# Julian-Wyatt/AnoDDPM

Measured on AMD Instinct MI355X. Metric: reverse-diffusion images/sec @256x256 T=1000 simplex, higher is better.
Workload: dtype f32; 1 GPU; 256x256 simplex(8 oct) T=1000 base128 attn16,8 batch4/GPU (BASELINE config 2); per_gpu_batch=4, global_batch=4, T=1000, parallelism=batch-sharded x1 (no data-path collective), output_finite=True

## Files before the change

anoddpm_amd/csrc/common.h:

```cpp
#pragma once
#include <hip/hip_runtime.h>
#include <stdint.h>
#include <stdio.h>
#include "../../include/anoddpm_hip.h"

namespace anoddpm {

void set_error(const char *fmt, ...);
extern int g_debug[16];

#define ANODDPM_REQUIRE(cond, ...)                       \
    do {                                                 \
        if (!(cond)) {                                   \
            ::anoddpm::set_error(__VA_ARGS__);           \
            return ANODDPM_EINVAL;                       \
        }                                                \
    } while (0)

inline int check_launch(const char *what)
{
    hipError_t e = hipGetLastError();
    if (e != hipSuccess) {
        set_error("%s: %s", what, hipGetErrorString(e));
        return ANODDPM_ELAUNCH;
    }
    return ANODDPM_OK;
}

constexpr int ANODDPM_MAX_DEV = 64;
inline int allow_big_lds(const void *fn, bool *done, const char *what)
{
    int dev = 0;
    if (hipGetDevice(&dev) != hipSuccess || dev < 0 || dev >= ANODDPM_MAX_DEV) dev = -1;
    if (dev >= 0 && done[dev]) return ANODDPM_OK;
    hipError_t e = hipFuncSetAttribute(fn, hipFuncAttributeMaxDynamicSharedMemorySize, 160 * 1024);
    if (e != hipSuccess) {
        set_error("%s: hipFuncSetAttribute(MaxDynamicSharedMemorySize): %s", what, hipGetErrorString(e));
        return ANODDPM_ELAUNCH;
    }
    if (dev >= 0) done[dev] = true;
    return ANODDPM_OK;
}

int launch_winograd(const anoddpm_igemm_args *a, hipStream_t s);
int launch_winograd43(const anoddpm_igemm_args *a, hipStream_t s);
int launch_winograd43r(const anoddpm_igemm_args *a, hipStream_t s);
int launch_winograd43w(const anoddpm_igemm_args *a, hipStream_t s, int tsplit);
int launch_pointwise_stream(const anoddpm_igemm_args *a, hipStream_t s);
int launch_smallmap(const anoddpm_igemm_args *a, hipStream_t s);
int smallmap_tile(int ks, int H, int W, int K, int c0, int N, int B);
int launch_wino23s(const anoddpm_igemm_args *a, hipStream_t s);
int launch_winograd43b(const anoddpm_igemm_args *a, hipStream_t s);
int wino23s_tile(int H, int W, int K, int c0, int N, int B, int a_mode);
int launch_wgrad43(const anoddpm_wgrad_args *a, hipStream_t s);
int wgrad43_groups(int K, int N, int B, int H, int W);
int wgrad43_colsum_items(int K, int N, int B, int H, int W);

inline hipStream_t as_stream(void *s) { return reinterpret_cast<hipStream_t>(s); }

__device__ __forceinline__ float silu_f(float x)
{
    return x * __builtin_amdgcn_rcpf(1.0f + __expf(-x));
}

}
```

anoddpm_amd/csrc/winograd43.hip:

```cpp
#include "common.h"
#include "gn_fold.h"

using anoddpm::silu_f;

namespace {

typedef float f32x4 __attribute__((ext_vector_type(4)));

constexpr int F4_NT = 768;
constexpr int F4_KC = 16;
constexpr int F4_PW = 18;
constexpr int F4_PPIX = F4_PW * F4_PW;
constexpr int F4_PITCH = 5;
constexpr int F4_PJ = 2;
constexpr int F4_SLOTPX = F4_PJ * F4_NT / 4;
constexpr int F4_DT = F4_SLOTPX * F4_PITCH;
constexpr int F4_V = 36 * 16 * 4;
constexpr int F4_MS = 52;
constexpr int F4_LOOP_FLOATS = (2 * F4_DT + 2 * F4_V) * 4;
constexpr int F4_EX_FLOATS = 36 * 16 * F4_MS;
constexpr int F4_LDS_FLOATS = F4_EX_FLOATS > F4_LOOP_FLOATS ? F4_EX_FLOATS : F4_LOOP_FLOATS;
constexpr int F4_KMAX = 1024;
constexpr int F4_AFF_FLOATS = 2 * F4_KMAX;

// ... 318 lines not shown
    };
    float rv[ROUNDS][16], add[ROUNDS], cs[ROUNDS], cq[ROUNDS];
    prefetch(item_of(0), rv[0], add[0]);
#pragma unroll
    for (int round = 0; round < ROUNDS; ++round) {
        const int nt0 = round * RT;
        const int ntn = (NTL == 8 && round == 2) ? 2 : RT;
#pragma unroll
        for (int p = 0; p < 3; ++p)
#pragma unroll
            for (int nt = 0; nt < 3; ++nt)
                if (nt < ntn) {
#pragma unroll
                    for (int r = 0; r < 4; ++r)
                        M[((wave * 3 + p) * 16 + kq * 4 + r) * F4_MS + nt * 16 + l15] = acc[p][nt0 + nt][r];
                }
        __syncthreads();
        if (round + 1 < ROUNDS) prefetch(item_of(round + 1), rv[round + 1], add[round + 1]);
        const Item it = item_of(round);
        cs[round] = 0.f;
        cq[round] = 0.f;
        if (it.active) {
            const float *m = M + (size_t)it.tile * F4_MS + it.ch;
            float y[4][6];
#pragma unroll
            for (int v = 0; v < 6; ++v) {
                float mu[6];
#pragma unroll
                for (int u = 0; u < 6; ++u) mu[u] = m[(size_t)((u * 6 + v) * 16) * F4_MS];
                const float s12 = mu[1] + mu[2], d12 = mu[1] - mu[2], s34 = mu[3] + mu[4], d34 = mu[3] - mu[4];
                y[0][v] = mu[0] + s12 + s34;
                y[1][v] = d12 + 2.f * d34;
                y[2][v] = s12 + 4.f * s34;
                y[3][v] = d12 + 8.f * d34 + mu[5];
            }
#pragma unroll
            for (int i = 0; i < 4; ++i) {
                const float s12 = y[i][1] + y[i][2], d12 = y[i][1] - y[i][2], s34 = y[i][3] + y[i][4], d34 = y[i][3] - y[i][4];
                float o4[4];
                o4[0] = y[i][0] + s12 + s34;
                o4[1] = d12 + 2.f * d34;
                o4[2] = s12 + 4.f * s34;
                o4[3] = d12 + 8.f * d34 + y[i][5];
#pragma unroll
                for (int j = 0; j < 4; ++j) {
                    const unsigned so = ((unsigned)i * uW + (unsigned)j) * 4u;
                    const float v = a.alpha * o4[j] + add[round] + rv[round][i * 4 + j];
                    __builtin_amdgcn_raw_buffer_store_b32(__builtin_bit_cast(unsigned, v), rO, (int)it.vo, (int)(so * o_ld), 0);
                    cs[round] += v;
                    cq[round] += v * v;
                }
            }
        }
        __syncthreads();
    }
    if (a.stats || a.stats_csum) {
        float *rs = M, *rq = M + ROUNDS * 16 * 48;
#pragma unroll
        for (int round = 0; round < ROUNDS; ++round) {
            const Item it = item_of(round);
            if (it.active) { rs[(round * 16 + it.tile) * 48 + it.ch] = cs[round]; rq[(round * 16 + it.tile) * 48 + it.ch] = cq[round]; }
        }
        __syncthreads();
        if (tid < NTL * 16) {
            const int round = tid / (RT * 16), chl = tid - round * (RT * 16);
            float s = 0.f, q = 0.f;
#pragma unroll
            for (int t = 0; t < 16; ++t) { s += rs[(round * 16 + t) * 48 + chl]; q += rq[(round * 16 + t) * 48 + chl]; }
            if (a.stats_csum) {
                anoddpm::csum_atomic_add(a.stats_csum, b, N, n0 + tid, s, q);
            } else {
                float *st = a.stats + (((int64_t)b * gridDim.x + blockIdx.x) * N + n0 + tid) * 2;
                st[0] = s;
                st[1] = q;
            }
        }
    }
}

}

extern "C" int anoddpm_f43_channel_sliced(int32_t H, int32_t W, int32_t N, int32_t B);

namespace anoddpm {

int launch_winograd43(const anoddpm_igemm_args *a, hipStream_t s)
{
    ANODDPM_REQUIRE(a->ks == 3 && a->b_mode == 0 && a->heads == 1, "winograd43: needs a 3x3 conv with packed weights");
    ANODDPM_REQUIRE(a->ksplit == 1 || (a->N % 128 == 0 && a->ws && (int64_t)a->B * a->ksplit <= 65535), "winograd43: split-K needs N %% 128 == 0 and a workspace");
    ANODDPM_REQUIRE(a->a_mode == 0 || a->a_mode == 1, "winograd43: pooled operand loads use the direct kernel");
    ANODDPM_REQUIRE(a->H % 16 == 0 && a->W % 16 == 0 && a->N % 64 == 0, "winograd43: H, W must be multiples of 16 and N of 64");
    const int K = a->c0 + a->c1;
    ANODDPM_REQUIRE(K % F4_KC == 0 && (a->c1 == 0 || a->c0 % F4_KC == 0), "winograd43: channel counts must be multiples of 16");
    ANODDPM_REQUIRE((int64_t)36 * K * a->N * 4 < ((int64_t)1 << 31), "winograd43: transformed weights exceed 32-bit buffer offsets");
    ANODDPM_REQUIRE(!(a->gn_scale || a->fold_gamma) || K <= F4_KMAX, "winograd43: the GroupNorm affine table holds %d input channels", F4_KMAX);
    if (a->fold_gamma) {
        ANODDPM_REQUIRE(a->fold_beta && a->fold_stats0 && (a->c1 == 0 || a->fold_stats1) && a->fold_fmt0 == 1 && (a->c1 == 0 || a->fold_fmt1 == 1),
                        "winograd43: the GroupNorm fold takes fp64 sums (fold_fmt 1: stats_csum / tail_csum sources) only");
        ANODDPM_REQUIRE(a->fold_groups >= 1 && a->fold_groups <= 64 && K % a->fold_groups == 0 && a->ksplit == 1,
                        "winograd43: GroupNorm fold: bad group count, or split-K");
        ANODDPM_REQUIRE(((uintptr_t)a->fold_stats0 | (uintptr_t)a->fold_stats1 | (uintptr_t)a->fold_gamma | (uintptr_t)a->fold_beta) % 16 == 0,
                        "winograd43: GroupNorm fold: sums, gamma and beta must be 16-byte aligned");
    }
    if (a->stats_csum)
        ANODDPM_REQUIRE(!a->stats && a->ksplit == 1 && a->heads == 1, "winograd43: stats_csum excludes stats rows, split-K and heads");
    ANODDPM_REQUIRE((int64_t)a->H * a->W * (a->a0_ld > a->a1_ld ? a->a0_ld : a->a1_ld) * 4 < ((int64_t)1 << 31),
                    "winograd43: operand slice exceeds 32-bit buffer offsets");
    const int64_t wg128 = (int64_t)(a->H / 16) * (a->W / 16) * (a->N / 128) * a->B;
    const bool half = (a->N % 128 != 0) || ((2 * wg128 + 255) / 256) * 71 < ((wg128 + 255) / 256) * 100;
    ANODDPM_REQUIRE(!a->gnb_partial || (a->ksplit == 1 && anoddpm_f43_channel_sliced(a->H, a->W, a->N, a->B) == 1),
                    "winograd43: gnb_partial needs the channel-sliced 128-channel kernel (anoddpm_f43_channel_sliced) and ksplit 1");
    const int nblk = half ? 64 : 128;
    dim3 grid((unsigned)((a->H / 16) * (a->W / 16)), (unsigned)(a->N / nblk), (unsigned)a->B);
    ANODDPM_REQUIRE(a->B <= 65535, "winograd43: batch too large");
    const bool fast = (a->gn_scale || a->fold_gamma) && a->act;
    ANODDPM_REQUIRE(a->res_mode == 0 || (a->res_mode == 1 && a->res && a->ksplit == 1), "winograd43: res_mode 1 needs a residual and ksplit 1");
#ifdef ANODDPM_ABLATE
    const int dbg = anoddpm::g_debug[2];
#else
    const int dbg = 0;
#endif
    if (a->ksplit > 1) {
        const int K16 = K / F4_KC, cps = (K16 + a->ksplit - 1) / a->ksplit;
        ANODDPM_REQUIRE((a->ksplit - 1) * cps < K16, "winograd43: ksplit leaves a slice without channels");
        return launch_winograd43r(a, s);
    }
    {
        const int v5 = anoddpm::g_debug[5];
        if (dbg == 0 && a->N % 128 == 0 && ((!half && (v5 == 4 || v5 == 5 || v5 == 8 || v5 == 9)) || v5 == 6 || v5 == 7))
            return launch_winograd43w(a, s, (v5 & 1) | (v5 >= 8 ? 2 : 0));
    }
    if (dbg == 0 && ((!half && anoddpm::g_debug[5] != 1) || (a->N % 128 == 0 && anoddpm::g_debug[5] == 3))) return launch_winograd43r(a, s);
#ifdef ANODDPM_ABLATE
    if (fast && dbg == 1) hipLaunchKernelGGL((wino43_kernel<true, 1>), grid, dim3(F4_NT), 0, s, *a);
    else if (fast && dbg == 2) hipLaunchKernelGGL((wino43_kernel<true, 2>), grid, dim3(F4_NT), 0, s, *a);
    else if (fast && dbg == 3) hipLaunchKernelGGL((wino43_kernel<true, 3>), grid, dim3(F4_NT), 0, s, *a);
    else if (fast && dbg == 4) hipLaunchKernelGGL((wino43_kernel<true, 4>), grid, dim3(F4_NT), 0, s, *a);
    else
#endif
    ANODDPM_REQUIRE(half || !a->fold_gamma, "winograd43: the position-sliced 128-channel kernel (ANODDPM_DEBUG5=1) does not fold the GroupNorm");
    if (fast && half) hipLaunchKernelGGL((wino43_kernel<true, 0, 4>), grid, dim3(F4_NT), 0, s, *a);
    else if (half) hipLaunchKernelGGL((wino43_kernel<false, 0, 4>), grid, dim3(F4_NT), 0, s, *a);
    else if (fast) hipLaunchKernelGGL((wino43_kernel<true>), grid, dim3(F4_NT), 0, s, *a);
    else      hipLaunchKernelGGL((wino43_kernel<false>), grid, dim3(F4_NT), 0, s, *a);
    return check_launch("winograd43");
}

}

extern "C" int anoddpm_f43_channel_sliced(int32_t H, int32_t W, int32_t N, int32_t B)
{
    if (H <= 0 || W <= 0 || N <= 0 || B <= 0 || H % 16 || W % 16 || N % 128) return 0;
    const int64_t wg128 = (int64_t)(H / 16) * (W / 16) * (N / 128) * B;
    const bool half = ((2 * wg128 + 255) / 256) * 71 < ((wg128 + 255) / 256) * 100;
    const int v5 = anoddpm::g_debug[5];
#ifdef ANODDPM_ABLATE
    if (anoddpm::g_debug[2] != 0) return 0;
#endif
    return ((!half && v5 == 0) || v5 == 3) ? 1 : 0;
}
```

anoddpm_amd/csrc/winograd43r.hip:

```cpp
#include <type_traits>

#include "common.h"
#include "gn_fold.h"

using anoddpm::silu_f;

namespace {

typedef float f32x4 __attribute__((ext_vector_type(4)));
typedef float f32x2 __attribute__((ext_vector_type(2)));
typedef unsigned u32x4 __attribute__((ext_vector_type(4)));

constexpr int R4_NT = 512;
constexpr int R4_KC = 16;
constexpr int R4_PW = 18;
constexpr int R4_PPIX = R4_PW * R4_PW;
constexpr int R4_PITCH = 5;
constexpr int R4_PJ = 3;
constexpr int R4_SLOTPX = R4_PJ * R4_NT / 4;
constexpr int R4_DT = R4_SLOTPX * R4_PITCH;
constexpr int R4_V = 36 * 16 * 4;
constexpr int R4_KMAX = 1024;
constexpr int R4_AFF = 2 * R4_KMAX / 4;
constexpr int R4_LDS_FLOATS = (2 * R4_DT + 2 * R4_V + R4_AFF) * 4;

__device__ __forceinline__ __amdgpu_buffer_rsrc_t rsrc(const float *base)
{
    return __builtin_amdgcn_make_buffer_rsrc(const_cast<float *>(base), 0, 0x7ffffffe, 0x00020000);
}
__device__ __forceinline__ f32x4 bld4(__amdgpu_buffer_rsrc_t r, unsigned lane_bytes, unsigned wave_bytes)
{
    return __builtin_bit_cast(f32x4, __builtin_amdgcn_raw_buffer_load_b128(r, (int)lane_bytes, (int)wave_bytes, 0));
}
template <int AUX>
__device__ __forceinline__ f32x4 bld4x(__amdgpu_buffer_rsrc_t r, unsigned lane_bytes, unsigned wave_bytes)
{
    return __builtin_bit_cast(f32x4, __builtin_amdgcn_raw_buffer_load_b128(r, (int)lane_bytes, (int)wave_bytes, AUX));
}

__device__ __forceinline__ void at6(const float (&m)[6], float (&o)[4])
{
    const float s12 = m[1] + m[2], d12 = m[1] - m[2], s34 = m[3] + m[4], d34 = m[3] - m[4];
    o[0] = m[0] + s12 + s34;
    o[1] = d12 + 2.f * d34;
    o[2] = s12 + 4.f * s34;
    o[3] = d12 + 8.f * d34 + m[5];
}

#ifndef F43_PAIR_TRANSFORM
#define F43_PAIR_TRANSFORM 0
#endif
constexpr int R4_VAR = F43_PAIR_TRANSFORM ? 32 : 0;
template <bool FAST, int DBG = 0, int R4_RING = 6, int NPOS = 36, int VAR = 0, bool GNB = false>
__global__ __launch_bounds__(R4_NT, 1) void wino43r_kernel(const anoddpm_igemm_args a)
{
    constexpr bool V_DEPHASE = (VAR & 1) != 0, V_SCALAR_T = (VAR & 2) != 0;
    constexpr bool V_PAIRS = (VAR & 32) != 0;
    constexpr bool V_PAIR = (VAR & 4) != 0, V_PRIO = (VAR & 8) != 0;
    constexpr int PATCH_AUX = (DBG == 18 || DBG == 19 || DBG == 21) ? 2 : 0;
    constexpr int RES_AUX = (DBG == 19 || DBG == 21) ? 2 : 0;
    constexpr int STORE_AUX = DBG == 19 ? 2 : ((DBG == 20 || DBG == 21) ? 16 : 0);
    unsigned long long tstamp[5];
    if (DBG == 5 || DBG == 6) tstamp[0] = __builtin_amdgcn_s_memtime();
    __shared__ __attribute__((aligned(16))) float lds[R4_LDS_FLOATS];
    f32x4 *ldsD = reinterpret_cast<f32x4 *>(lds);
    f32x4 *ldsV = ldsD + 2 * R4_DT;
    f32x4 *ldsAff = ldsV + 2 * R4_V;

    const int tid = threadIdx.x, lane = tid & 63;
    const int wave = __builtin_amdgcn_readfirstlane(tid >> 6);
    const int H = a.H, W = a.W;
    const int K = a.c0 + a.c1, N = a.N, K4 = K >> 2;
    const int tiles_x = W >> 4;
    int tile = blockIdx.x;
    if ((VAR & 16) && (gridDim.x & 7) == 0) tile = (blockIdx.x & 7) * (gridDim.x >> 3) + (blockIdx.x >> 3);
    const int y0 = (tile / tiles_x) * 16, x0 = (tile % tiles_x) * 16;
    const int n0 = blockIdx.y * 128;
    const int ksplit = a.ksplit;
    const int ksi = blockIdx.z % ksplit;
    const int b = blockIdx.z / ksplit;
    const int a_mode = a.a_mode;

    const float *A0 = a.a0 + (int64_t)b * a.a0_bs;
    const float *A1 = a.a1 ? a.a1 + (int64_t)b * a.a1_bs : nullptr;
    const float *gsc = a.gn_scale ? a.gn_scale + (int64_t)b * a.gn_ld : nullptr;
    const float *gsh = a.gn_shift ? a.gn_shift + (int64_t)b * a.gn_ld : nullptr;
    const bool fold = a.fold_gamma != nullptr;
    const bool affine = gsc != nullptr || fold, act = a.act != 0;
    const int cps = (K / R4_KC + ksplit - 1) / ksplit;
    const int cb = ksi * cps;
    const int nchunks = (cb + cps <= K / R4_KC ? cps : K / R4_KC - cb);

    int spix[R4_PJ];
    const int pq = tid & 3;
#pragma unroll
    for (int j = 0; j < R4_PJ; ++j) {
        const int p = (tid + j * R4_NT) >> 2;
        const int py = p / R4_PW, px = p - py * R4_PW;
        const int gy = y0 + py - 1, gx = x0 + px - 1;
        int sp = -1;
        if (p < R4_PPIX && gy >= 0 && gy < H && gx >= 0 && gx < W)
            sp = (a_mode == 0) ? gy * W + gx : (gy >> 1) * (W >> 1) + (gx >> 1);
        spix[j] = sp;
    }
    f32x4 praw[R4_PJ];
    f32x4 asc = {1.f, 1.f, 1.f, 1.f}, ash = {0.f, 0.f, 0.f, 0.f};
    const __amdgpu_buffer_rsrc_t rA0 = rsrc(A0), rA1 = rsrc(A1 ? A1 : A0);
    const __amdgpu_buffer_rsrc_t rSc = rsrc(gsc ? gsc : A0), rSh = rsrc(gsh ? gsh : A0);
    auto load_patch = [&](int chunk) {
        const int kbase = (cb + chunk) * R4_KC;
        const bool first = kbase < a.c0;
        const __amdgpu_buffer_rsrc_t r = first ? rA0 : rA1;
        const unsigned ld = (unsigned)(first ? a.a0_ld : a.a1_ld);
        const unsigned koff = (unsigned)(first ? kbase : kbase - a.c0) * 4u;
#pragma unroll
        for (int j = 0; j < R4_PJ; ++j) {
            const unsigned sp = (DBG == 7) ? (unsigned)(y0 * W + x0) : (spix[j] >= 0 ? (unsigned)spix[j] : 0u);
            praw[j] = bld4x<PATCH_AUX>(r, (sp * ld + (unsigned)(pq * 4)) * 4u, koff);
        }
    };
    auto store_patch = [&](int buf, int chunk) {
        const f32x4 zero = {0.f, 0.f, 0.f, 0.f};
        if (FAST || affine) {
            asc = ldsAff[(cb + chunk) * 4 + pq];
            ash = ldsAff[K4 + (cb + chunk) * 4 + pq];
        }
#pragma unroll
        for (int j = 0; j < R4_PJ; ++j) {
            const int idx = tid + j * R4_NT;
            f32x4 v = praw[j];
            if (DBG == 22) {
                const f32x4 same = {0.25f, -0.5f, 0.75f, 1.0f};
                v = (praw[j][0] == 12345.678f) ? praw[j] : same;
            }
            if (FAST) {
                v = v * asc + ash;
                v[0] = silu_f(v[0]); v[1] = silu_f(v[1]); v[2] = silu_f(v[2]); v[3] = silu_f(v[3]);
            } else {
                if (affine) v = v * asc + ash;
                if (act) { v[0] = silu_f(v[0]); v[1] = silu_f(v[1]); v[2] = silu_f(v[2]); v[3] = silu_f(v[3]); }
            }
            ldsD[buf * R4_DT + (idx >> 2) * R4_PITCH + (idx & 3)] = spix[j] >= 0 ? v : zero;
        }
    };

    const int tu = wave % 6;
    const int tpair = lane & 7;
    const int ttile = ((wave / 6) * 2 + (lane >> 5)) * 4 + ((lane >> 3) & 3);
    const int tbase2 = (((4 * (ttile >> 2)) * R4_PW + 4 * (ttile & 3)) * R4_PITCH) * 2 + tpair;
    const bool two_pass = wave >= 2 && wave <= 5;
    constexpr int PASS_D = 8 * R4_PW * R4_PITCH * 2;
    constexpr int PASS_V = 8 * 8;
    const int tr0 = (tu == 0) ? 0 : 1, tr1 = (tu == 5) ? 3 : 2, tr2 = (tu == 0) ? 4 : ((tu == 5) ? 5 : 3), tr3 = 4;
    const float tc0 = (tu == 0) ? 4.f : (tu == 1 ? -4.f : (tu == 2 ? 4.f : (tu == 3 ? -2.f : (tu == 4 ? 2.f : 4.f))));
    const float tc1 = (tu == 0 || tu == 5) ? -5.f : ((tu == 1 || tu == 2) ? -4.f : -1.f);
    const float tc2 = (tu == 0 || tu == 5) ? 1.f : (tu == 1 ? 1.f : (tu == 2 ? -1.f : (tu == 3 ? 2.f : -2.f)));
    const float tc3 = (tu == 0 || tu == 5) ? 0.f : 1.f;
    const int to0 = tr0 * R4_PW * R4_PITCH * 2, to1 = tr1 * R4_PW * R4_PITCH * 2, to2 = tr2 * R4_PW * R4_PITCH * 2, to3 = tr3 * R4_PW * R4_PITCH * 2;
    auto transform = [&](int pbuf, int vbuf, int dofs, int vofs) {
        const f32x2 *D = reinterpret_cast<const f32x2 *>(ldsD + pbuf * R4_DT) + tbase2 + dofs;
// ... 9 lines not shown
        V[3 * 128] = r + 2.f * s;
        V[4 * 128] = r - 2.f * s;
        V[5 * 128] = 4.f * t[1] - 5.f * t[3] + t[5];
    };
    auto transform_s = [&](int pbuf, int vbuf, int dofs, int vofs) {
        const f32x2 *D = reinterpret_cast<const f32x2 *>(ldsD + pbuf * R4_DT) + tbase2 + dofs;
        float tx[6], ty[6];
#pragma unroll
        for (int j = 0; j < 6; ++j) {
            const f32x2 d0 = D[to0 + j * R4_PITCH * 2], d1 = D[to1 + j * R4_PITCH * 2], d2 = D[to2 + j * R4_PITCH * 2], d3 = D[to3 + j * R4_PITCH * 2];
            tx[j] = tc0 * d0[0] + tc1 * d1[0] + tc2 * d2[0] + tc3 * d3[0];
            ty[j] = tc0 * d0[1] + tc1 * d1[1] + tc2 * d2[1] + tc3 * d3[1];
        }
        f32x2 *V = reinterpret_cast<f32x2 *>(ldsV + vbuf * R4_V) + ((tu * 6) * 16 + ttile) * 8 + tpair + vofs;
        const float px = tx[4] - 4.f * tx[2], qx = tx[3] - 4.f * tx[1], rx = tx[4] - tx[2], sx = tx[3] - tx[1];
        const float py = ty[4] - 4.f * ty[2], qy = ty[3] - 4.f * ty[1], ry = ty[4] - ty[2], sy = ty[3] - ty[1];
        V[0 * 128] = f32x2{4.f * tx[0] - 5.f * tx[2] + tx[4], 4.f * ty[0] - 5.f * ty[2] + ty[4]};
        V[1 * 128] = f32x2{px + qx, py + qy};
        V[2 * 128] = f32x2{px - qx, py - qy};
        V[3 * 128] = f32x2{rx + 2.f * sx, ry + 2.f * sy};
        V[4 * 128] = f32x2{rx - 2.f * sx, ry - 2.f * sy};
        V[5 * 128] = f32x2{4.f * tx[1] - 5.f * tx[3] + tx[5], 4.f * ty[1] - 5.f * ty[3] + ty[5]};
    };
    const int p_up = wave % 3;
    const int p_tx = lane >> 4, p_ch = lane & 15;
    constexpr int PP = R4_PITCH * 4, PROW = R4_PW * PP;
    const int p_in = ((4 * (wave / 3)) * R4_PW + 4 * p_tx) * PP + p_ch;
    const int p_out = ((wave / 3) * 4 + p_tx) * 16 + p_ch;
    const int p_ua = p_up == 0 ? 0 : (p_up == 1 ? 1 : 3), p_ub = p_up == 0 ? 5 : (p_up == 1 ? 2 : 4);
    constexpr int PASS_DP = 8 * PROW, PASS_VP = 2 * 4 * 16;
    auto col_pass = [&](const float (&t)[6], float *V) {
        const float p = t[4] - 4.f * t[2], q = t[3] - 4.f * t[1], r = t[4] - t[2], w = t[3] - t[1];
        V[0 * 256] = 4.f * t[0] - 5.f * t[2] + t[4];
        V[1 * 256] = p + q;
        V[2 * 256] = p - q;
        V[3 * 256] = r + 2.f * w;
        V[4 * 256] = r - 2.f * w;
        V[5 * 256] = 4.f * t[1] - 5.f * t[3] + t[5];
    };
    auto transform_p = [&](int pbuf, int vbuf, int dofs, int vofs) {
        const float *D = reinterpret_cast<const float *>(ldsD + pbuf * R4_DT) + p_in + dofs;
        float ta[6], tb[6];
        if (p_up == 0) {
#pragma unroll
            for (int j = 0; j < 6; ++j) {
                const float d0 = D[j * PP], d1 = D[PROW + j * PP], d2 = D[2 * PROW + j * PP], d3 = D[3 * PROW + j * PP], d4 = D[4 * PROW + j * PP], d5 = D[5 * PROW + j * PP];
                ta[j] = 4.f * d0 - 5.f * d2 + d4;
                tb[j] = 4.f * d1 - 5.f * d3 + d5;
            }
        } else if (p_up == 1) {
#pragma unroll
            for (int j = 0; j < 6; ++j) {
                const float d1 = D[PROW + j * PP], d2 = D[2 * PROW + j * PP], d3 = D[3 * PROW + j * PP], d4 = D[4 * PROW + j * PP];
                const float p = d4 - 4.f * d2, q = d3 - 4.f * d1;
                ta[j] = p + q;
                tb[j] = p - q;
            }
        } else {
#pragma unroll
            for (int j = 0; j < 6; ++j) {
                const float d1 = D[PROW + j * PP], d2 = D[2 * PROW + j * PP], d3 = D[3 * PROW + j * PP], d4 = D[4 * PROW + j * PP];
                const float r = d4 - d2, w = d3 - d1;
                ta[j] = r + 2.f * w;
                tb[j] = r - 2.f * w;
            }
        }
        float *V = reinterpret_cast<float *>(ldsV + vbuf * R4_V) + p_out + vofs;
        col_pass(ta, V + p_ua * 6 * 256);
        col_pass(tb, V + p_ub * 6 * 256);
    };
    auto transform_all = [&](int pbuf, int vbuf) {
        if (V_PAIRS) {
            transform_p(pbuf, vbuf, 0, 0);
            if (two_pass) transform_p(pbuf, vbuf, PASS_DP, PASS_VP);
        } else if (V_SCALAR_T) {
            transform_s(pbuf, vbuf, 0, 0);
            if (two_pass) transform_s(pbuf, vbuf, PASS_D, PASS_V);
        } else {
            transform(pbuf, vbuf, 0, 0);
            if (two_pass) transform(pbuf, vbuf, PASS_D, PASS_V);
        }
    };

    f32x4 acc[NPOS];
#pragma unroll
    for (int p = 0; p < NPOS; ++p) acc[p] = f32x4{0.f, 0.f, 0.f, 0.f};

    const int l15 = lane & 15, kq = lane >> 4;
    const int nw = n0 + wave * 16 + l15;
    const __amdgpu_buffer_rsrc_t rU = rsrc(a.bmat);
    const unsigned xi_bytes = (unsigned)K4 * (unsigned)N * 16u;
    const unsigned ulane = ((unsigned)kq * (unsigned)N + (unsigned)nw) * 16u;
    const int vread = l15 * 4 + kq;

    f32x4 ring[R4_RING];
    auto load_b = [&](int chunk, int pos, int slot) {
        ring[slot] = bld4(rU, ulane, (unsigned)pos * xi_bytes + (unsigned)((cb + chunk) * 4) * (unsigned)N * 16u);
    };

    const int last = nchunks - 1;
    const int c1 = last >= 1 ? 1 : 0, c2 = last >= 2 ? 2 : last;
    f32x4 aff_sc = {0.f, 0.f, 0.f, 0.f}, aff_sh = {0.f, 0.f, 0.f, 0.f};
    const bool aff_slot = (FAST || affine) && tid < K4 && !fold;
    anoddpm::FoldLoads fl;
    if (aff_slot) {
        aff_sc = bld4(rSc, (unsigned)(tid * 16), 0u);
        aff_sh = bld4(rSh, (unsigned)(tid * 16), 0u);
    } else if (fold) {
        fl = anoddpm::fold_affine_request(a, b, tid);
    }
    load_patch(0);
    f32x4 praw0[R4_PJ];
#pragma unroll
    for (int j = 0; j < R4_PJ; ++j) praw0[j] = praw[j];
    load_patch(c1);
#pragma unroll
    for (int g = 0; g < R4_RING; ++g) load_b(0, g, g);
    if (FAST || affine) {
        if (fold) {
            anoddpm::fold_affine_finish(a, fl, tid, a_mode == 1 ? (H >> 1) * (W >> 1) : H * W, reinterpret_cast<double *>(ldsV), ldsAff);
        } else if (aff_slot) {
            ldsAff[tid] = aff_sc;
            ldsAff[K4 + tid] = aff_sh;
        }
        __syncthreads();
    }
    {
        f32x4 keep[R4_PJ];
#pragma unroll
        for (int j = 0; j < R4_PJ; ++j) { keep[j] = praw[j]; praw[j] = praw0[j]; }
        store_patch(0, 0);
#pragma unroll
        for (int j = 0; j < R4_PJ; ++j) praw[j] = keep[j];
    }
    __syncthreads();
    transform_all(0, 0);
    store_patch(1, c1);
    load_patch(c2);
    __syncthreads();
    if (DBG == 5 || DBG == 6) tstamp[1] = __builtin_amdgcn_s_memtime();

    auto step = [&](const int chunk, auto doT, auto doS, auto doL, auto doR, auto &&res_prefetch) {
        if (decltype(doT)::value && DBG != 2 && !(V_DEPHASE && wave >= 4)) transform_all((chunk + 1) & 1, (chunk + 1) & 1);
        const f32x4 *V = ldsV + (chunk & 1) * R4_V + vread;
        constexpr int PS = NPOS / 4, PL = 3 * NPOS / 4, PR = NPOS - 6;
        if (V_PAIR) {
            f32x4 av4[4];
            av4[0] = V[0];
            av4[1] = V[64];
#pragma unroll
            for (int p = 0; p < NPOS; p += 2) {
                if (V_DEPHASE && p == NPOS / 2 && decltype(doT)::value && wave >= 4) transform_all((chunk + 1) & 1, (chunk + 1) & 1);
                if ((p == PS || p == PS + 1) && decltype(doS)::value) store_patch(chunk & 1, chunk + 2);
                if ((p == PL || p == PL + 1) && decltype(doL)::value) load_patch(chunk + 3);
                if ((p == PR || p == PR + 1) && decltype(doR)::value) res_prefetch();
                const f32x4 a0 = av4[p % 4], a1 = av4[(p + 1) % 4];
                if (p + 2 < NPOS) { av4[(p + 2) % 4] = V[(p + 2) * 64]; av4[(p + 3) % 4] = V[(p + 3) * 64]; }
                const f32x4 b0 = ring[p % R4_RING], b1 = ring[(p + 1) % R4_RING];
#pragma unroll
                for (int kk = 0; kk < 4; ++kk) {
                    acc[p] = __builtin_amdgcn_mfma_f32_16x16x4f32(a0[kk], b0[kk], acc[p], 0, 0, 0);
                    acc[p + 1] = __builtin_amdgcn_mfma_f32_16x16x4f32(a1[kk], b1[kk], acc[p + 1], 0, 0, 0);
                }
#pragma unroll
                for (int q = p; q < p + 2; ++q) {
                    if (q + R4_RING < NPOS)           load_b(chunk, q + R4_RING, q % R4_RING);
                    else if (!decltype(doR)::value)   load_b(chunk + 1, q + R4_RING - NPOS, q % R4_RING);
                }
                __builtin_amdgcn_sched_barrier(0);
            }
            if (!decltype(doR)::value) __syncthreads();
            return;
        }
        f32x4 av[3];
        av[0] = V[0];
        av[1] = V[64];
#pragma unroll
        for (int p = 0; p < NPOS; ++p) {
            if (V_DEPHASE && p == NPOS / 2 && decltype(doT)::value && wave >= 4) transform_all((chunk + 1) & 1, (chunk + 1) & 1);
            if (p == PS && decltype(doS)::value && DBG != 3 && DBG != 11) store_patch(chunk & 1, chunk + 2);
            if (p == PL && decltype(doL)::value && DBG != 3) load_patch(chunk + 3);
            if (p == PR && decltype(doR)::value) res_prefetch();
            const f32x4 a_cur = av[p % 3];
            if (p + 2 < NPOS && DBG != 23) av[(p + 2) % 3] = V[(p + 2) * 64];
            const f32x4 bv = ring[p % R4_RING];
#pragma unroll
            for (int kk = 0; kk < 4; ++kk)
                acc[p] = __builtin_amdgcn_mfma_f32_16x16x4f32(a_cur[kk], bv[kk], acc[p], 0, 0, 0);
            if (DBG != 4) {
                if (p + R4_RING < NPOS)           load_b(chunk, p + R4_RING, p % R4_RING);
                else if (!decltype(doR)::value)   load_b(chunk + 1, p + R4_RING - NPOS, p % R4_RING);
            }
            __builtin_amdgcn_sched_barrier(0);
        }
        if (!decltype(doR)::value) __syncthreads();
    };
    if (V_PRIO && wave >= 4) __builtin_amdgcn_s_setprio(1);
    constexpr std::true_type YES{};
    constexpr std::false_type NO{};
    auto nothing = []() {};
    int chunk = 0;
    for (; chunk + 3 <= last; ++chunk) step(chunk, YES, YES, YES, NO, nothing);

    const bool part = ksplit > 1;
    const float *TE = (a.temb && !part) ? a.temb + (int64_t)b * a.temb_ld : nullptr;
    const __amdgpu_buffer_rsrc_t rO = part ? rsrc(a.ws + ((int64_t)ksi * a.B + b) * ((int64_t)H * W * N))
                                           : rsrc(a.out + (int64_t)b * a.o_bs);
    const bool gx_first = !GNB || n0 + wave * 16 < a.gnb_c0;
    const float *gx = !GNB ? nullptr : (gx_first ? a.gnb_x0 + (int64_t)b * a.gnb_x0_bs : a.gnb_x1 + (int64_t)b * a.gnb_x1_bs);
    const __amdgpu_buffer_rsrc_t rR = GNB ? rsrc(gx) : rsrc(a.res ? a.res + (int64_t)b * a.r_bs : a.out);
    const bool has_res = GNB || (a.res != nullptr && !part);
    const unsigned uW = (unsigned)W, o_ld = part ? (unsigned)N : (unsigned)a.out_ld;
    const unsigned r_ld = GNB ? (unsigned)(gx_first ? a.gnb_x0_ld : a.gnb_x1_ld) : (unsigned)a.res_ld;
    const float alpha = part ? 1.0f : a.alpha;
    float add = 0.f;
    if (a.bias && !part) add += a.bias[nw];
    if (TE) add += TE[nw];
    const unsigned pix0 = (unsigned)(y0 + kq * 4) * uW + (unsigned)x0;
    const unsigned nwr = GNB ? (unsigned)(gx_first ? nw : nw - a.gnb_c0) : (unsigned)nw;
    const unsigned vo = (pix0 * o_ld + (unsigned)nw) * 4u, vr = (pix0 * r_ld + nwr) * 4u;
    const bool res_up = !GNB && a.res_mode == 1;
    const unsigned hW = uW >> 1;
    const unsigned vrh = ((((unsigned)(y0 + kq * 4) >> 1) * hW + ((unsigned)x0 >> 1)) * r_ld + nwr) * 4u;
    auto load_res = [&](int r, float (&rv)[16]) {
#pragma unroll
        for (int i = 0; i < 16; ++i) rv[i] = 0.f;
        if (DBG == 24) return;
        if (has_res && res_up) {
#pragma unroll
            for (int i2 = 0; i2 < 2; ++i2)
#pragma unroll
                for (int j2 = 0; j2 < 2; ++j2) {
                    const float v = __builtin_bit_cast(float, __builtin_amdgcn_raw_buffer_load_b32(
                        rR, (int)vrh, (int)((((unsigned)(r * 2) + (unsigned)i2 * hW + (unsigned)j2) * 4u) * r_ld), RES_AUX));
                    rv[(2 * i2) * 4 + 2 * j2] = v; rv[(2 * i2) * 4 + 2 * j2 + 1] = v;
                    rv[(2 * i2 + 1) * 4 + 2 * j2] = v; rv[(2 * i2 + 1) * 4 + 2 * j2 + 1] = v;
                }
        } else if (has_res) {
#pragma unroll
            for (int i = 0; i < 4; ++i)
#pragma unroll
                for (int j = 0; j < 4; ++j)
                    rv[i * 4 + j] = __builtin_bit_cast(float, __builtin_amdgcn_raw_buffer_load_b32(
                        rR, (int)vr, (int)((((unsigned)(r * 4) + (unsigned)i * uW + (unsigned)j) * 4u) * r_ld), RES_AUX));
        }
    };
    float rv[2][16];
    if (last >= 2) step(last - 2, YES, YES, NO, NO, nothing);
    if (last >= 1) step(last - 1, YES, NO, NO, NO, nothing);
    step(last, NO, NO, NO, YES, [&]() { load_res(0, rv[0]); });

    if (DBG == 5 || DBG == 6) tstamp[2] = __builtin_amdgcn_s_memtime();
    if (DBG == 1 || NPOS < 36) {
        float sum = 0.f;
#pragma unroll
        for (int p = 0; p < NPOS; ++p) sum += (acc[p][0] + acc[p][1]) + (acc[p][2] + acc[p][3]);
        if (sum == 12345.678f) a.out[0] = sum;
        return;
    }
    float cs = 0.f, cq = 0.f;
    float g_sc = 0.f, g_sh = 0.f, g_mu = 0.f, g_rs = 0.f;
    if (GNB) {
        const int grp = nw / (N / a.gnb_groups);
        g_mu = a.gnb_mean[(int64_t)b * a.gnb_groups + grp];
        g_rs = a.gnb_rstd[(int64_t)b * a.gnb_groups + grp];
        g_sc = a.gnb_gamma[nw] * g_rs;
        g_sh = a.gnb_beta[nw] - g_mu * g_sc;
    }
#pragma unroll
    for (int r = 0; r < 4; ++r) {
        if (r + 1 < 4) load_res(r + 1, rv[(r + 1) & 1]);
        float y[4][6];
#pragma unroll
        for (int v = 0; v < 6; ++v) {
            float mu[6], o[4];
#pragma unroll
            for (int u = 0; u < 6; ++u) mu[u] = acc[u * 6 + v][r];
            at6(mu, o);
#pragma unroll
            for (int i = 0; i < 4; ++i) y[i][v] = o[i];
        }
#pragma unroll
        for (int i = 0; i < 4; ++i) {
            float o4[4];
            at6(y[i], o4);
#pragma unroll
            for (int j = 0; j < 4; ++j) {
                const unsigned so = ((unsigned)(r * 4) + (unsigned)i * uW + (unsigned)j) * 4u;
                const float v = GNB ? alpha * o4[j] + add : alpha * o4[j] + add + rv[r & 1][i * 4 + j];
                if (DBG != 25 || (r == 0 && i == 0 && j == 0))
                    __builtin_amdgcn_raw_buffer_store_b32(__builtin_bit_cast(unsigned, v), rO, (int)vo, (int)(so * o_ld), STORE_AUX);
                if (GNB) {
                    const float x = rv[r & 1][i * 4 + j];
                    const float y = x * g_sc + g_sh;
                    const float sg = __builtin_amdgcn_rcpf(1.0f + __expf(-y));
                    const float dyv = v * (sg * (1.0f + y * (1.0f - sg)));
                    cs += dyv;
                    cq += dyv * ((x - g_mu) * g_rs);
                } else {
                    cs += v;
                    cq += v * v;
                }
            }
        }
    }
    if (GNB) {
        cs += __shfl_xor(cs, 16);
        cq += __shfl_xor(cq, 16);
        cs += __shfl_xor(cs, 32);
        cq += __shfl_xor(cq, 32);
        if (kq == 0) {
            double *pp = a.gnb_partial + (((int64_t)b * gridDim.x + tile) * N + nw) * 2;
            pp[0] = (double)cs;
            pp[1] = (double)cq;
        }
    } else if ((a.stats || a.stats_csum) && !part) {
        cs += __shfl_xor(cs, 16);
        cq += __shfl_xor(cq, 16);
        cs += __shfl_xor(cs, 32);
        cq += __shfl_xor(cq, 32);
        if (kq == 0) {
            if (a.stats_csum) {
                anoddpm::csum_atomic_add(a.stats_csum, b, N, nw, cs, cq);
            } else {
                float *st = a.stats + (((int64_t)b * gridDim.x + blockIdx.x) * N + nw) * 2;
                st[0] = cs;
                st[1] = cq;
            }
        }
    }
    if (DBG == 5 || DBG == 6) {
        tstamp[3] = __builtin_amdgcn_s_memtime();
        if (DBG == 5) __builtin_amdgcn_s_waitcnt(0);
        tstamp[4] = __builtin_amdgcn_s_memtime();
        if (tid == 0) {
            unsigned long long *d = reinterpret_cast<unsigned long long *>(a.ws) +
                                    (((int64_t)blockIdx.z * gridDim.y + blockIdx.y) * gridDim.x + blockIdx.x) * 8;
#pragma unroll
            for (int i = 0; i < 5; ++i) d[i] = tstamp[i];
            d[5] = (unsigned long long)__builtin_amdgcn_s_getreg(63492);
            d[6] = (unsigned long long)__builtin_amdgcn_s_getreg(63508);
            d[7] = 0;
        }
    }
}

}

namespace anoddpm {

int launch_winograd43r(const anoddpm_igemm_args *a, hipStream_t s)
{
    dim3 grid((unsigned)((a->H / 16) * (a->W / 16)), (unsigned)(a->N / 128), (unsigned)(a->B * a->ksplit));
    const bool fast = (a->gn_scale || a->fold_gamma) && a->act;
    ANODDPM_REQUIRE(!(a->gn_scale || a->fold_gamma) || a->c0 + a->c1 <= R4_KMAX, "winograd43r: GroupNorm affine table holds %d input channels", R4_KMAX);
#ifdef ANODDPM_ABLATE
    const int dbg = g_debug[6];
    if (fast && dbg == 1) hipLaunchKernelGGL((wino43r_kernel<true, 1>), grid, dim3(R4_NT), 0, s, *a);
    else if (fast && dbg == 2) hipLaunchKernelGGL((wino43r_kernel<true, 2>), grid, dim3(R4_NT), 0, s, *a);
    else if (fast && dbg == 3) hipLaunchKernelGGL((wino43r_kernel<true, 3>), grid, dim3(R4_NT), 0, s, *a);
    else if (fast && dbg == 4) hipLaunchKernelGGL((wino43r_kernel<true, 4>), grid, dim3(R4_NT), 0, s, *a);
    else if (fast && dbg == 5) hipLaunchKernelGGL((wino43r_kernel<true, 5>), grid, dim3(R4_NT), 0, s, *a);
    else if (fast && dbg == 6) hipLaunchKernelGGL((wino43r_kernel<true, 6>), grid, dim3(R4_NT), 0, s, *a);
    else if (fast && dbg == 7) hipLaunchKernelGGL((wino43r_kernel<true, 7, 9>), grid, dim3(R4_NT), 0, s, *a);
    else if (fast && dbg == 11) hipLaunchKernelGGL((wino43r_kernel<true, 11, 9>), grid, dim3(R4_NT), 0, s, *a);
    else if (fast && dbg == 12) hipLaunchKernelGGL((wino43r_kernel<true, 3, 9>), grid, dim3(R4_NT), 0, s, *a);
    else if (fast && dbg == 13) hipLaunchKernelGGL((wino43r_kernel<true, 4, 9>), grid, dim3(R4_NT), 0, s, *a);
    else if (fast && dbg == 24) hipLaunchKernelGGL((wino43r_kernel<true, 24, 9>), grid, dim3(R4_NT), 0, s, *a);
    else if (fast && dbg == 25) hipLaunchKernelGGL((wino43r_kernel<true, 25, 9>), grid, dim3(R4_NT), 0, s, *a);
    else if (fast && dbg == 23) hipLaunchKernelGGL((wino43r_kernel<true, 23, 9>), grid, dim3(R4_NT), 0, s, *a);
    else if (fast && dbg == 22) hipLaunchKernelGGL((wino43r_kernel<true, 22, 9>), grid, dim3(R4_NT), 0, s, *a);
    else if (fast && dbg == 18) hipLaunchKernelGGL((wino43r_kernel<true, 18, 9>), grid, dim3(R4_NT), 0, s, *a);
    else if (fast && dbg == 19) hipLaunchKernelGGL((wino43r_kernel<true, 19, 9>), grid, dim3(R4_NT), 0, s, *a);
    else if (fast && dbg == 20) hipLaunchKernelGGL((wino43r_kernel<true, 20, 9>), grid, dim3(R4_NT), 0, s, *a);
    else if (fast && dbg == 21) hipLaunchKernelGGL((wino43r_kernel<true, 21, 9>), grid, dim3(R4_NT), 0, s, *a);
    else if (fast && dbg == 14) hipLaunchKernelGGL((wino43r_kernel<true, 0, 9, 18>), grid, dim3(R4_NT), 0, s, *a);
    else if (fast && dbg == 15) hipLaunchKernelGGL((wino43r_kernel<true, 0, 18, 18>), grid, dim3(R4_NT), 0, s, *a);
    else if (fast && dbg == 16) hipLaunchKernelGGL((wino43r_kernel<true, 7, 9, 18>), grid, dim3(R4_NT), 0, s, *a);
    else if (fast && dbg == 17) hipLaunchKernelGGL((wino43r_kernel<true, 0, 6, 18>), grid, dim3(R4_NT), 0, s, *a);
    else if (fast && dbg == 8) hipLaunchKernelGGL((wino43r_kernel<true, 0, 8>), grid, dim3(R4_NT), 0, s, *a);
    else if (fast && dbg == 10) hipLaunchKernelGGL((wino43r_kernel<true, 0, 6>), grid, dim3(R4_NT), 0, s, *a);
    else if (fast && dbg == 9) hipLaunchKernelGGL((wino43r_kernel<true, 0, 4>), grid, dim3(R4_NT), 0, s, *a);
    else if (fast && dbg == 30) hipLaunchKernelGGL((wino43r_kernel<true, 0, 9, 36, 1>), grid, dim3(R4_NT), 0, s, *a);
    else if (fast && dbg == 31) hipLaunchKernelGGL((wino43r_kernel<true, 0, 9, 36, 2>), grid, dim3(R4_NT), 0, s, *a);
    else if (fast && dbg == 32) hipLaunchKernelGGL((wino43r_kernel<true, 0, 9, 36, 3>), grid, dim3(R4_NT), 0, s, *a);
    else if (fast && dbg == 33) hipLaunchKernelGGL((wino43r_kernel<true, 0, 6, 36, 1>), grid, dim3(R4_NT), 0, s, *a);
    else if (fast && dbg == 34) hipLaunchKernelGGL((wino43r_kernel<true, 0, 6, 36, 3>), grid, dim3(R4_NT), 0, s, *a);
    else if (fast && dbg == 39) hipLaunchKernelGGL((wino43r_kernel<true, 0, 9, 36, 16>), grid, dim3(R4_NT), 0, s, *a);
    else if (fast && dbg == 35) hipLaunchKernelGGL((wino43r_kernel<true, 0, 6, 36, 4>), grid, dim3(R4_NT), 0, s, *a);
    else if (fast && dbg == 36) hipLaunchKernelGGL((wino43r_kernel<true, 0, 6, 36, 5>), grid, dim3(R4_NT), 0, s, *a);
    else if (fast && dbg == 37) hipLaunchKernelGGL((wino43r_kernel<true, 0, 9, 36, 8>), grid, dim3(R4_NT), 0, s, *a);
    else if (fast && dbg == 38) hipLaunchKernelGGL((wino43r_kernel<true, 0, 9, 36, 9>), grid, dim3(R4_NT), 0, s, *a);
    else if (fast && dbg == 40) hipLaunchKernelGGL((wino43r_kernel<true, 0, 9, 36, 32>), grid, dim3(R4_NT), 0, s, *a);
    else if (fast && dbg == 41) hipLaunchKernelGGL((wino43r_kernel<true, 0, 12, 36, 32>), grid, dim3(R4_NT), 0, s, *a);
    else
#endif
    if (a->gnb_partial) {
        ANODDPM_REQUIRE(!fast && !a->gn_scale && !a->fold_gamma && !a->act && a->ksplit == 1 && !a->res && !a->bias && !a->temb && !a->stats && !a->stats_csum,
                        "winograd43r: gnb_partial needs a plain data-gradient launch (no gn / act / bias / temb / res / stats, ksplit 1)");
        ANODDPM_REQUIRE(a->gnb_x0 && a->gnb_gamma && a->gnb_beta && a->gnb_mean && a->gnb_rstd && a->gnb_groups > 0 && a->N % a->gnb_groups == 0 &&
                        a->gnb_c0 > 0 && a->gnb_c0 % 16 == 0 && a->gnb_c0 <= a->N && (a->gnb_c0 == a->N || a->gnb_x1),
                        "winograd43r: gnb_partial: bad GroupNorm arguments");
        ANODDPM_REQUIRE((int64_t)a->H * a->W * (a->gnb_x0_ld > a->gnb_x1_ld ? a->gnb_x0_ld : a->gnb_x1_ld) * 4 < ((int64_t)1 << 31),
                        "winograd43r: gnb_partial: source slice exceeds 32-bit buffer offsets");
        hipLaunchKernelGGL((wino43r_kernel<false, 0, 6, 36, R4_VAR, true>), grid, dim3(R4_NT), 0, s, *a);
        return check_launch("winograd43r");
    }
    if (fast) hipLaunchKernelGGL((wino43r_kernel<true, 0, 9, 36, R4_VAR>), grid, dim3(R4_NT), 0, s, *a);
    else      hipLaunchKernelGGL((wino43r_kernel<false, 0, 6, 36, R4_VAR>), grid, dim3(R4_NT), 0, s, *a);
    return check_launch("winograd43r");
}

}
```

Before: 0.4466 images/s.

## Add 64-channel workgroup variant of register-blocked Winograd F(4,3) kernel

Adds an NB=64 form of the wino43r kernel. The eight waves split into two phases, each covering half of the 36 Winograd positions for 16 channels. Partial accumulators are exchanged through LDS before the output transform, and the GroupNorm stats partials are combined the same way. The half-grid case, previously routed to the older wino43 kernel, now uses this variant by default. The aim is more workgroups to fill CUs when layers are small, at the cost of an extra LDS exchange and two syncs.

```diff
diff --git a/anoddpm_amd/csrc/common.h b/anoddpm_amd/csrc/common.h
--- a/anoddpm_amd/csrc/common.h
+++ b/anoddpm_amd/csrc/common.h
@@ -44,7 +44,7 @@
 
 int launch_winograd(const anoddpm_igemm_args *a, hipStream_t s);
 int launch_winograd43(const anoddpm_igemm_args *a, hipStream_t s);
-int launch_winograd43r(const anoddpm_igemm_args *a, hipStream_t s);
+int launch_winograd43r(const anoddpm_igemm_args *a, hipStream_t s, int nblk = 128);
 int launch_winograd43w(const anoddpm_igemm_args *a, hipStream_t s, int tsplit);
 int launch_pointwise_stream(const anoddpm_igemm_args *a, hipStream_t s);
 int launch_smallmap(const anoddpm_igemm_args *a, hipStream_t s);
diff --git a/anoddpm_amd/csrc/winograd43.hip b/anoddpm_amd/csrc/winograd43.hip
--- a/anoddpm_amd/csrc/winograd43.hip
+++ b/anoddpm_amd/csrc/winograd43.hip
@@ -424,6 +424,17 @@
 
 extern "C" int anoddpm_f43_channel_sliced(int32_t H, int32_t W, int32_t N, int32_t B);
 
+namespace {
+
+constexpr int F43_HALF_COST = 71;
+
+bool f43_half_grid(int64_t wg128)
+{
+    return ((2 * wg128 + 255) / 256) * F43_HALF_COST < ((wg128 + 255) / 256) * 100;
+}
+
+}
+
 namespace anoddpm {
 
 int launch_winograd43(const anoddpm_igemm_args *a, hipStream_t s)
@@ -449,7 +460,7 @@
     ANODDPM_REQUIRE((int64_t)a->H * a->W * (a->a0_ld > a->a1_ld ? a->a0_ld : a->a1_ld) * 4 < ((int64_t)1 << 31),
                     "winograd43: operand slice exceeds 32-bit buffer offsets");
     const int64_t wg128 = (int64_t)(a->H / 16) * (a->W / 16) * (a->N / 128) * a->B;
-    const bool half = (a->N % 128 != 0) || ((2 * wg128 + 255) / 256) * 71 < ((wg128 + 255) / 256) * 100;
+    const bool half = (a->N % 128 != 0) || f43_half_grid(wg128);
     ANODDPM_REQUIRE(!a->gnb_partial || (a->ksplit == 1 && anoddpm_f43_channel_sliced(a->H, a->W, a->N, a->B) == 1),
                     "winograd43: gnb_partial needs the channel-sliced 128-channel kernel (anoddpm_f43_channel_sliced) and ksplit 1");
     const int nblk = half ? 64 : 128;
@@ -472,7 +483,11 @@
         if (dbg == 0 && a->N % 128 == 0 && ((!half && (v5 == 4 || v5 == 5 || v5 == 8 || v5 == 9)) || v5 == 6 || v5 == 7))
             return launch_winograd43w(a, s, (v5 & 1) | (v5 >= 8 ? 2 : 0));
     }
-    if (dbg == 0 && ((!half && anoddpm::g_debug[5] != 1) || (a->N % 128 == 0 && anoddpm::g_debug[5] == 3))) return launch_winograd43r(a, s);
+    {
+        const int v5 = anoddpm::g_debug[5];
+        if (dbg == 0 && ((!half && v5 != 1 && v5 != 11) || (a->N % 128 == 0 && v5 == 3))) return launch_winograd43r(a, s);
+        if (dbg == 0 && ((half && v5 != 1 && v5 != 10) || v5 == 11)) return launch_winograd43r(a, s, 64);
+    }
 #ifdef ANODDPM_ABLATE
     if (fast && dbg == 1) hipLaunchKernelGGL((wino43_kernel<true, 1>), grid, dim3(F4_NT), 0, s, *a);
     else if (fast && dbg == 2) hipLaunchKernelGGL((wino43_kernel<true, 2>), grid, dim3(F4_NT), 0, s, *a);
@@ -494,7 +509,7 @@
 {
     if (H <= 0 || W <= 0 || N <= 0 || B <= 0 || H % 16 || W % 16 || N % 128) return 0;
     const int64_t wg128 = (int64_t)(H / 16) * (W / 16) * (N / 128) * B;
-    const bool half = ((2 * wg128 + 255) / 256) * 71 < ((wg128 + 255) / 256) * 100;
+    const bool half = f43_half_grid(wg128);
     const int v5 = anoddpm::g_debug[5];
 #ifdef ANODDPM_ABLATE
     if (anoddpm::g_debug[2] != 0) return 0;
diff --git a/anoddpm_amd/csrc/winograd43r.hip b/anoddpm_amd/csrc/winograd43r.hip
--- a/anoddpm_amd/csrc/winograd43r.hip
+++ b/anoddpm_amd/csrc/winograd43r.hip
@@ -51,9 +51,14 @@
 #define F43_PAIR_TRANSFORM 0
 #endif
 constexpr int R4_VAR = F43_PAIR_TRANSFORM ? 32 : 0;
-template <bool FAST, int DBG = 0, int R4_RING = 6, int NPOS = 36, int VAR = 0, bool GNB = false>
+constexpr int R4_RING64 = 9;
+template <bool FAST, int DBG = 0, int R4_RING = 6, int NPOS = 36, int VAR = 0, bool GNB = false, int NB = 128>
 __global__ __launch_bounds__(R4_NT, 1) void wino43r_kernel(const anoddpm_igemm_args a)
 {
+    static_assert(NB == 128 || (NB == 64 && DBG == 0 && NPOS == 36 && (VAR & ~32) == 0 && !GNB),
+                  "the 64-channel workgroup has no ablation, measurement-variant or GNB form");
+    constexpr int LP = NB == 64 ? NPOS / 2 : NPOS;
+    static_assert(NB == 128 || LP % R4_RING == 0, "the B ring depth must divide the positions of a wave");
     constexpr bool V_DEPHASE = (VAR & 1) != 0, V_SCALAR_T = (VAR & 2) != 0;
     constexpr bool V_PAIRS = (VAR & 32) != 0;
     constexpr bool V_PAIR = (VAR & 4) != 0, V_PRIO = (VAR & 8) != 0;
@@ -75,7 +80,9 @@
     int tile = blockIdx.x;
     if ((VAR & 16) && (gridDim.x & 7) == 0) tile = (blockIdx.x & 7) * (gridDim.x >> 3) + (blockIdx.x >> 3);
     const int y0 = (tile / tiles_x) * 16, x0 = (tile % tiles_x) * 16;
-    const int n0 = blockIdx.y * 128;
+    const int n0 = blockIdx.y * NB;
+    const int cw = NB == 64 ? (wave & 3) : wave;
+    const int ph = NB == 64 ? (wave >> 2) : 0;
     const int ksplit = a.ksplit;
     const int ksi = blockIdx.z % ksplit;
     const int b = blockIdx.z / ksplit;
@@ -251,20 +258,20 @@
         }
     };
 
-    f32x4 acc[NPOS];
-#pragma unroll
-    for (int p = 0; p < NPOS; ++p) acc[p] = f32x4{0.f, 0.f, 0.f, 0.f};
+    f32x4 acc[LP];
+#pragma unroll
+    for (int p = 0; p < LP; ++p) acc[p] = f32x4{0.f, 0.f, 0.f, 0.f};
 
     const int l15 = lane & 15, kq = lane >> 4;
-    const int nw = n0 + wave * 16 + l15;
+    const int nw = n0 + cw * 16 + l15;
     const __amdgpu_buffer_rsrc_t rU = rsrc(a.bmat);
     const unsigned xi_bytes = (unsigned)K4 * (unsigned)N * 16u;
     const unsigned ulane = ((unsigned)kq * (unsigned)N + (unsigned)nw) * 16u;
-    const int vread = l15 * 4 + kq;
+    const int vread = ph * (LP * 64) + l15 * 4 + kq;
 
     f32x4 ring[R4_RING];
     auto load_b = [&](int chunk, int pos, int slot) {
-        ring[slot] = bld4(rU, ulane, (unsigned)pos * xi_bytes + (unsigned)((cb + chunk) * 4) * (unsigned)N * 16u);
+        ring[slot] = bld4(rU, ulane, (unsigned)(ph * LP + pos) * xi_bytes + (unsigned)((cb + chunk) * 4) * (unsigned)N * 16u);
     };
 
     const int last = nchunks - 1;
@@ -312,19 +319,19 @@
     auto step = [&](const int chunk, auto doT, auto doS, auto doL, auto doR, auto &&res_prefetch) {
         if (decltype(doT)::value && DBG != 2 && !(V_DEPHASE && wave >= 4)) transform_all((chunk + 1) & 1, (chunk + 1) & 1);
         const f32x4 *V = ldsV + (chunk & 1) * R4_V + vread;
-        constexpr int PS = NPOS / 4, PL = 3 * NPOS / 4, PR = NPOS - 6;
+        constexpr int PS = LP / 4, PL = 3 * LP / 4, PR = LP - 6;
         if (V_PAIR) {
             f32x4 av4[4];
             av4[0] = V[0];
             av4[1] = V[64];
 #pragma unroll
-            for (int p = 0; p < NPOS; p += 2) {
-                if (V_DEPHASE && p == NPOS / 2 && decltype(doT)::value && wave >= 4) transform_all((chunk + 1) & 1, (chunk + 1) & 1);
+            for (int p = 0; p < LP; p += 2) {
+                if (V_DEPHASE && p == LP / 2 && decltype(doT)::value && wave >= 4) transform_all((chunk + 1) & 1, (chunk + 1) & 1);
                 if ((p == PS || p == PS + 1) && decltype(doS)::value) store_patch(chunk & 1, chunk + 2);
                 if ((p == PL || p == PL + 1) && decltype(doL)::value) load_patch(chunk + 3);
                 if ((p == PR || p == PR + 1) && decltype(doR)::value) res_prefetch();
                 const f32x4 a0 = av4[p % 4], a1 = av4[(p + 1) % 4];
-                if (p + 2 < NPOS) { av4[(p + 2) % 4] = V[(p + 2) * 64]; av4[(p + 3) % 4] = V[(p + 3) * 64]; }
+                if (p + 2 < LP) { av4[(p + 2) % 4] = V[(p + 2) * 64]; av4[(p + 3) % 4] = V[(p + 3) * 64]; }
                 const f32x4 b0 = ring[p % R4_RING], b1 = ring[(p + 1) % R4_RING];
 #pragma unroll
                 for (int kk = 0; kk < 4; ++kk) {
@@ -333,8 +340,8 @@
                 }
 #pragma unroll
                 for (int q = p; q < p + 2; ++q) {
-                    if (q + R4_RING < NPOS)           load_b(chunk, q + R4_RING, q % R4_RING);
-                    else if (!decltype(doR)::value)   load_b(chunk + 1, q + R4_RING - NPOS, q % R4_RING);
+                    if (q + R4_RING < LP)             load_b(chunk, q + R4_RING, q % R4_RING);
+                    else if (!decltype(doR)::value)   load_b(chunk + 1, q + R4_RING - LP, q % R4_RING);
                 }
                 __builtin_amdgcn_sched_barrier(0);
             }
@@ -345,20 +352,20 @@
         av[0] = V[0];
         av[1] = V[64];
 #pragma unroll
-        for (int p = 0; p < NPOS; ++p) {
-            if (V_DEPHASE && p == NPOS / 2 && decltype(doT)::value && wave >= 4) transform_all((chunk + 1) & 1, (chunk + 1) & 1);
+        for (int p = 0; p < LP; ++p) {
+            if (V_DEPHASE && p == LP / 2 && decltype(doT)::value && wave >= 4) transform_all((chunk + 1) & 1, (chunk + 1) & 1);
             if (p == PS && decltype(doS)::value && DBG != 3 && DBG != 11) store_patch(chunk & 1, chunk + 2);
             if (p == PL && decltype(doL)::value && DBG != 3) load_patch(chunk + 3);
             if (p == PR && decltype(doR)::value) res_prefetch();
             const f32x4 a_cur = av[p % 3];
-            if (p + 2 < NPOS && DBG != 23) av[(p + 2) % 3] = V[(p + 2) * 64];
+            if (p + 2 < LP && DBG != 23) av[(p + 2) % 3] = V[(p + 2) * 64];
             const f32x4 bv = ring[p % R4_RING];
 #pragma unroll
             for (int kk = 0; kk < 4; ++kk)
                 acc[p] = __builtin_amdgcn_mfma_f32_16x16x4f32(a_cur[kk], bv[kk], acc[p], 0, 0, 0);
             if (DBG != 4) {
-                if (p + R4_RING < NPOS)           load_b(chunk, p + R4_RING, p % R4_RING);
-                else if (!decltype(doR)::value)   load_b(chunk + 1, p + R4_RING - NPOS, p % R4_RING);
+                if (p + R4_RING < LP)             load_b(chunk, p + R4_RING, p % R4_RING);
+                else if (!decltype(doR)::value)   load_b(chunk + 1, p + R4_RING - LP, p % R4_RING);
             }
             __builtin_amdgcn_sched_barrier(0);
         }
@@ -417,16 +424,50 @@
     float rv[2][16];
     if (last >= 2) step(last - 2, YES, YES, NO, NO, nothing);
     if (last >= 1) step(last - 1, YES, NO, NO, NO, nothing);
-    step(last, NO, NO, NO, YES, [&]() { load_res(0, rv[0]); });
+    constexpr int NR = NB == 64 ? 2 : 4;
+    const int r0 = ph * NR;
+    step(last, NO, NO, NO, YES, [&]() { load_res(r0, rv[0]); });
 
     if (DBG == 5 || DBG == 6) tstamp[2] = __builtin_amdgcn_s_memtime();
     if (DBG == 1 || NPOS < 36) {
         float sum = 0.f;
 #pragma unroll
-        for (int p = 0; p < NPOS; ++p) sum += (acc[p][0] + acc[p][1]) + (acc[p][2] + acc[p][3]);
+        for (int p = 0; p < LP; ++p) sum += (acc[p][0] + acc[p][1]) + (acc[p][2] + acc[p][3]);
         if (sum == 12345.678f) a.out[0] = sum;
         return;
     }
+    float m2[NB == 64 ? 36 : 1][2];
+    if constexpr (NB == 64) {
+        f32x2 *xb = reinterpret_cast<f32x2 *>(lds);
+        __syncthreads();
+        if (ph == 0) {
+#pragma unroll
+            for (int p = 0; p < LP; ++p) xb[(wave * LP + p) * 64 + lane] = f32x2{acc[p][2], acc[p][3]};
+        } else {
+#pragma unroll
+            for (int p = 0; p < LP; ++p) xb[(wave * LP + p) * 64 + lane] = f32x2{acc[p][0], acc[p][1]};
+        }
+        __syncthreads();
+        if (ph == 0) {
+#pragma unroll
+            for (int p = 0; p < LP; ++p) {
+                const f32x2 o = xb[((wave ^ 4) * LP + p) * 64 + lane];
+                m2[p][0] = acc[p][0]; m2[p][1] = acc[p][1];
+                m2[LP + p][0] = o[0]; m2[LP + p][1] = o[1];
+            }
+        } else {
+#pragma unroll
+            for (int p = 0; p < LP; ++p) {
+                const f32x2 o = xb[((wave ^ 4) * LP + p) * 64 + lane];
+                m2[p][0] = o[0]; m2[p][1] = o[1];
+                m2[LP + p][0] = acc[p][2]; m2[LP + p][1] = acc[p][3];
+            }
+        }
+    }
+    auto m_at = [&](int pos, int rr) -> float {
+        if constexpr (NB == 64) return m2[pos][rr];
+        else return acc[pos][rr];
+    };
     float cs = 0.f, cq = 0.f;
     float g_sc = 0.f, g_sh = 0.f, g_mu = 0.f, g_rs = 0.f;
     if (GNB) {
@@ -437,14 +478,15 @@
         g_sh = a.gnb_beta[nw] - g_mu * g_sc;
     }
 #pragma unroll
-    for (int r = 0; r < 4; ++r) {
-        if (r + 1 < 4) load_res(r + 1, rv[(r + 1) & 1]);
+    for (int rr = 0; rr < NR; ++rr) {
+        const int r = r0 + rr;
+        if (rr + 1 < NR) load_res(r + 1, rv[(rr + 1) & 1]);
         float y[4][6];
 #pragma unroll
         for (int v = 0; v < 6; ++v) {
             float mu[6], o[4];
 #pragma unroll
-            for (int u = 0; u < 6; ++u) mu[u] = acc[u * 6 + v][r];
+            for (int u = 0; u < 6; ++u) mu[u] = m_at(u * 6 + v, rr);
             at6(mu, o);
 #pragma unroll
             for (int i = 0; i < 4; ++i) y[i][v] = o[i];
@@ -456,11 +498,11 @@
 #pragma unroll
             for (int j = 0; j < 4; ++j) {
                 const unsigned so = ((unsigned)(r * 4) + (unsigned)i * uW + (unsigned)j) * 4u;
-                const float v = GNB ? alpha * o4[j] + add : alpha * o4[j] + add + rv[r & 1][i * 4 + j];
-                if (DBG != 25 || (r == 0 && i == 0 && j == 0))
+                const float v = GNB ? alpha * o4[j] + add : alpha * o4[j] + add + rv[rr & 1][i * 4 + j];
+                if (DBG != 25 || (rr == 0 && i == 0 && j == 0))
                     __builtin_amdgcn_raw_buffer_store_b32(__builtin_bit_cast(unsigned, v), rO, (int)vo, (int)(so * o_ld), STORE_AUX);
                 if (GNB) {
-                    const float x = rv[r & 1][i * 4 + j];
+                    const float x = rv[rr & 1][i * 4 + j];
                     const float y = x * g_sc + g_sh;
                     const float sg = __builtin_amdgcn_rcpf(1.0f + __expf(-y));
                     const float dyv = v * (sg * (1.0f + y * (1.0f - sg)));
@@ -488,7 +530,17 @@
         cq += __shfl_xor(cq, 16);
         cs += __shfl_xor(cs, 32);
         cq += __shfl_xor(cq, 32);
-        if (kq == 0) {
+        if constexpr (NB == 64) {
+            f32x2 *sf = reinterpret_cast<f32x2 *>(ldsAff);
+            if (ph == 1 && kq == 0) sf[cw * 16 + l15] = f32x2{cs, cq};
+            __syncthreads();
+            if (ph == 0 && kq == 0) {
+                const f32x2 o = sf[cw * 16 + l15];
+                cs += o[0];
+                cq += o[1];
+            }
+        }
+        if (kq == 0 && ph == 0) {
             if (a.stats_csum) {
                 anoddpm::csum_atomic_add(a.stats_csum, b, N, nw, cs, cq);
             } else {
@@ -518,11 +570,18 @@
 
 namespace anoddpm {
 
-int launch_winograd43r(const anoddpm_igemm_args *a, hipStream_t s)
+int launch_winograd43r(const anoddpm_igemm_args *a, hipStream_t s, int nblk)
 {
-    dim3 grid((unsigned)((a->H / 16) * (a->W / 16)), (unsigned)(a->N / 128), (unsigned)(a->B * a->ksplit));
+    ANODDPM_REQUIRE(nblk == 128 || nblk == 64, "winograd43r: workgroups of 128 or 64 channels");
+    dim3 grid((unsigned)((a->H / 16) * (a->W / 16)), (unsigned)(a->N / nblk), (unsigned)(a->B * a->ksplit));
     const bool fast = (a->gn_scale || a->fold_gamma) && a->act;
     ANODDPM_REQUIRE(!(a->gn_scale || a->fold_gamma) || a->c0 + a->c1 <= R4_KMAX, "winograd43r: GroupNorm affine table holds %d input channels", R4_KMAX);
+    if (nblk == 64) {
+        ANODDPM_REQUIRE(a->ksplit == 1 && !a->gnb_partial, "winograd43r: the 64-channel workgroup has no split-K and no gnb_partial form");
+        if (fast) hipLaunchKernelGGL((wino43r_kernel<true, 0, R4_RING64, 36, R4_VAR, false, 64>), grid, dim3(R4_NT), 0, s, *a);
+        else      hipLaunchKernelGGL((wino43r_kernel<false, 0, R4_RING64, 36, R4_VAR, false, 64>), grid, dim3(R4_NT), 0, s, *a);
+        return check_launch("winograd43r");
+    }
 #ifdef ANODDPM_ABLATE
     const int dbg = g_debug[6];
     if (fast && dbg == 1) hipLaunchKernelGGL((wino43r_kernel<true, 1>), grid, dim3(R4_NT), 0, s, *a);
```

New measurement: 0.4489 images/s, median of 6. No clear change (+0.5%).
